# treangenlab/komb

Hardware: AMD Instinct MI355X
Metric: peeled edges/sec (k-truss) (higher is better)
Workload: dtype int32

## Files before the change

include/komb_accel.h:

```cpp
#ifndef KOMB_ACCEL_H
#define KOMB_ACCEL_H

#include <stdint.h>

#ifdef __cplusplus
extern "C" {
#endif

#define KOMB_ACCEL_ABI_VERSION 7

typedef enum komb_status {
    KOMB_OK          =  0,
    KOMB_ERR_ARG     = -1,
    KOMB_ERR_DEVICE  = -2,
    KOMB_ERR_NOMEM   = -3,
    KOMB_ERR_LIMIT   = -4,
    KOMB_ERR_STATE   = -5
} komb_status;

typedef struct komb_ctx komb_ctx;

typedef struct komb_opts {
    int32_t device;
    int32_t verbosity;
// ... 2 lines not shown
#define KOMB_CREATE_NULL_STREAM 1
#define KOMB_CREATE_NO_WARMUP   2
#define KOMB_CREATE_WARM_UPLOAD 4

typedef struct komb_stats {
    int64_t nv, ne;
    int64_t triangles;
    int64_t sum_deg_sq;
    int64_t wedge_items;
    int64_t oriented_items;
    int32_t max_degree, max_coreness, max_trussness;
    int32_t core_levels, core_subrounds;
    int32_t core_launches, truss_tail_runs;
    int32_t truss_levels, truss_subrounds;
    int32_t truss_scans, truss_launches;
    double  ms_build;
    double  ms_core;
    double  ms_orient;
    double  ms_tri_count;
    double  ms_tri_fill;
    double  ms_compact;
    double  ms_support;
    double  ms_allreduce;
    double  ms_peel;
    double  ms_gather;
    double  ms_corea;
    double  ms_tail;
    int64_t core_local_items, truss_local_items;
    int32_t core_local_units, core_local_sweeps;
    int32_t truss_local_units, truss_local_sweeps;
    double  ms_core_local;
    double  ms_truss_local;
    double  ms_sort;
    int64_t tri_records;
    int32_t index_layout;
    int32_t shard_exchanges;
    double  ms_exchange;
    int64_t exchange_words;
    double  ms_build_h2d;
    double  ms_build_relabel;
    double  ms_prepare;
    int32_t truss_prepared;
    int32_t engine_flags;
    double  ms_prep_vertex;
    double  ms_prep_edges;
    double  ms_prep_rows;
    int32_t stream_retries;
    int32_t reserved0;
} komb_stats;
#define KOMB_ENGINE_LOCAL_FINISH 1
#define KOMB_ENGINE_LDS_TAIL     2
#define KOMB_ENGINE_SHARD_PEEL   4
#define KOMB_ENGINE_TWO_PASS     8

komb_ctx   *komb_create(const komb_opts *opts);
void        komb_destroy(komb_ctx *ctx);
const char *komb_last_error(const komb_ctx *ctx);
int         komb_abi_version(void);
int         komb_set_option(komb_ctx *ctx, const char *name, const char *value);

int komb_graph_from_edges(komb_ctx *ctx, int64_t nv, int64_t n_raw,
                          const int64_t *uv_pairs);

int komb_graph_from_csr(komb_ctx *ctx, int64_t nv, const int64_t *rowptr,
                        const int32_t *col);

int komb_graph_info(komb_ctx *ctx, int64_t *nv, int64_t *ne);

int komb_graph_get_csr(komb_ctx *ctx, int64_t *rowptr, int32_t *col);

int komb_core_run(komb_ctx *ctx);
typedef int (*komb_allreduce_fn)(void *user, void *device_u32, int64_t count);
int komb_core_run_sharded(komb_ctx *ctx, int32_t rank, int32_t world, komb_allreduce_fn allreduce, void *user);
int komb_core_fetch(komb_ctx *ctx, int32_t *degree , int32_t *coreness );
int komb_degree_coreness(komb_ctx *ctx, int32_t *degree, int32_t *coreness);

int komb_onion_run(komb_ctx *ctx);
int komb_onion_fetch(komb_ctx *ctx, int32_t *layer , int32_t *coreness );
int komb_onion_info(komb_ctx *ctx, int64_t *n_layers, int32_t *max_coreness, double *ms);

#define KOMB_COMP_CORE   0
#define KOMB_COMP_TRUSS  1
#define KOMB_COMP_K_MAX (-1)
int komb_components_run(komb_ctx *ctx, int32_t kind, int32_t k);
int komb_components_fetch(komb_ctx *ctx, int32_t *label , int32_t *size );
int komb_components_info(komb_ctx *ctx, int32_t *kind, int32_t *k_used, int64_t *n_members,
                         int64_t *n_components, int64_t *largest, double *ms);

#define KOMB_COMM_K_MAX (-1)
int komb_truss_communities_run(komb_ctx *ctx, int32_t k);
int komb_truss_communities_fetch(komb_ctx *ctx, int32_t *label , int32_t *size );
int komb_truss_communities_fetch_vertices(komb_ctx *ctx, int32_t *n_comm );
int komb_truss_communities_info(komb_ctx *ctx, int32_t *k_used, int64_t *n_member_edges, int64_t *n_communities,
                                int64_t *largest, int64_t *n_multi_vertices, double *ms);

int komb_truss_run(komb_ctx *ctx, const uint8_t *vmask);
int komb_truss_prepare(komb_ctx *ctx);
int komb_truss_unprepare(komb_ctx *ctx);
int komb_truss_run_sharded(komb_ctx *ctx, const uint8_t *vmask, int32_t rank, int32_t world,
                           komb_allreduce_fn allreduce, void *user);
int komb_set_shard_peel(komb_ctx *ctx, int32_t on);
int komb_truss_run_slice(komb_ctx *ctx, const uint8_t *vmask, int32_t rank, int32_t world);
int komb_truss_count(komb_ctx *ctx, int64_t *ne_sub);
int komb_truss_fetch(komb_ctx *ctx, int32_t *eu, int32_t *ev, int32_t *truss);
int komb_truss_fetch_support(komb_ctx *ctx, int32_t *support);
int komb_trussness(komb_ctx *ctx, const uint8_t *vmask, int64_t *ne_out,
// ... 21 lines not shown
```

komb_amd/api.py:

```python
import ctypes
import os

import numpy as np

from . import _lib
from ._lib import KombOpts, KombStats, as_c, ptr


class KombError(RuntimeError):
    def __init__(self, code, msg):
        super().__init__(f"komb_accel error {code}: {msg}")
        self.code = code


def gen_hug_edges(nv, n_cliques, alpha=2.6, seed=42):
    lib = _lib.load()
    n_raw = lib.komb_gen_hug_edges(nv, n_cliques, alpha, seed, None)
    if n_raw < 0:
        raise ValueError("komb_gen_hug_edges: bad arguments")
    uv = np.empty((n_raw, 2), dtype=np.int64)
    got = lib.komb_gen_hug_edges(nv, n_cliques, alpha, seed, ptr(uv))
    assert got == n_raw
    return uv


FORWARD_ENV_OPTIONS = False
OPTION_NAMES = ("FINISH", "LOCAL_LIMIT", "LOCAL_ITEMS", "LOCAL_DENSITY", "LOCAL_DEFER_CHUNKS", "TAIL", "CORE_TAIL", "INDEX",
                "REC_CAP", "OWN_DENSE_CAP", "NO_OWN_DENSE", "NO_REC_SCRATCH", "NO_FIRST_QUEUE", "FULL_CAPS", "PREP_ROW_STAGE", "RETIRE_EVERY", "SHARD_ENGINE",
                "TRI_DEBUG", "POOL_DEBUG", "BUILD_DEBUG", "LOCAL_DEBUG", "TAIL_DEBUG", "COMP_SAMPLE", "COMM_SHORT", "COMM_HEAVY", "POISON")

SENTINEL_I32 = -0x5A5A5A5B


def _out_i32(n):
    return np.full(n, SENTINEL_I32, dtype=np.int32)


def _out_f64(n):
    return np.full(n, np.nan, dtype=np.float64)


class KombAccel:
    def __init__(self, device=0, verbosity=0, flags=0):
        self._lib = _lib.load()
        opts = KombOpts(device=device, verbosity=verbosity)
        opts.reserved[0] = flags
        self._ctx = self._lib.komb_create(ctypes.byref(opts))
        if not self._ctx:
            raise MemoryError("komb_create failed")
        self.device = device
        self.nv = -1
        self.ne = 0
        self._forwarded = {}

    def set_option(self, name, value):
        v = None if value is None else str(value).encode()
        self._check(self._lib.komb_set_option(self._ctx, name.encode(), v))

    def _sync_env_options(self):
        if not FORWARD_ENV_OPTIONS:
            return
        for name in OPTION_NAMES:
            v = os.environ.get("KOMB_" + name)
            if name == "INDEX" and os.environ.get("KOMB_TWO_PASS"):
                v = "two_pass"
            if name == "SHARD_ENGINE" and v is None:
                v = os.environ.get("KOMB_SHARD_PEEL")
            if self._forwarded.get(name) != v:
                self.set_option(name, v)
                self._forwarded[name] = v

    def close(self):
        if getattr(self, "_ctx", None):
            self._lib.komb_destroy(self._ctx)
            self._ctx = None

    def __del__(self):
        self.close()

    def __enter__(self):
# ... 203 lines not shown
```

komb_amd/csrc/api.cpp:

```cpp
#include "common.h"

#include <cerrno>
#include <cmath>
#include <cstdlib>
#include <cstring>
#include <memory>
#include <new>
#include <vector>

using namespace komb;

namespace {

int require_device(komb_ctx *ctx)
{
    if (!ctx) return KOMB_ERR_ARG;
    if (!ctx->device_ok) {
        if (ctx->err.empty()) ctx->err = "no usable HIP device";
        return KOMB_ERR_DEVICE;
    }
    KOMB_HIP(ctx, hipSetDevice(ctx->device));
    ctx->err.clear();
    return KOMB_OK;
}

}

extern "C" {

int komb_abi_version(void) { return KOMB_ACCEL_ABI_VERSION; }

komb_ctx *komb_create(const komb_opts *opts)
{
    komb_ctx *ctx = new (std::nothrow) komb_ctx();
    if (!ctx) return nullptr;
    if (opts) ctx->opts = *opts;
    ctx->device = ctx->opts.device;
    int ndev = 0;
    hipError_t e = hipGetDeviceCount(&ndev);
    if (e != hipSuccess || ndev <= 0) {
        ctx->err = std::string("no usable HIP device: ") + (e != hipSuccess ? hipGetErrorString(e) : "device count is 0");
        (void)hipGetLastError();
        return ctx;
    }
    if (ctx->device < 0 || ctx->device >= ndev) {
        ctx->err = "device ordinal out of range";
        return ctx;
    }
    e = hipSetDevice(ctx->device);
    if (e == hipSuccess) e = hipHostMalloc((void **)&ctx->h_ctrl, 2 * sizeof(PeelCtrl), hipHostMallocDefault);
    if (e == hipSuccess) e = hipHostMalloc((void **)&ctx->h_local, 2 * sizeof(LocalCtrl), hipHostMallocDefault);
    if (e == hipSuccess) e = hipHostMalloc(&ctx->h_stage, kStageBytes, hipHostMallocDefault);
    ctx->stream = nullptr;
    if (e == hipSuccess && !(ctx->opts.reserved[0] & KOMB_CREATE_NULL_STREAM)) { e = hipStreamCreate(&ctx->stream); ctx->own_stream = e == hipSuccess; }
    if (e == hipSuccess && !ctx->timer.init()) e = hipErrorUnknown;
    if (e != hipSuccess) {
        ctx->err = std::string("device initialisation failed: ") + hipGetErrorString(e);
        return ctx;
    }
    ctx->device_ok = true;
    if (!(ctx->opts.reserved[0] & KOMB_CREATE_NO_WARMUP)) warm_up(ctx);
    return ctx;
}

void komb_destroy(komb_ctx *ctx)
{
    if (!ctx) return;
    if (ctx->device_ok) {
        (void)hipSetDevice(ctx->device);
        graph_free(ctx);
        stager_free(ctx);
        ctx->pool.clear();
        ctx->timer.destroy();
        if (ctx->own_stream && ctx->stream) (void)hipStreamDestroy(ctx->stream);
        if (ctx->h_ctrl) (void)hipHostFree(ctx->h_ctrl);
        if (ctx->h_local) (void)hipHostFree(ctx->h_local);
        if (ctx->h_stage) (void)hipHostFree(ctx->h_stage);
    }
    delete ctx;
}

const char *komb_last_error(const komb_ctx *ctx) { return ctx ? ctx->err.c_str() : "null context"; }

int komb_graph_from_edges(komb_ctx *ctx, int64_t nv, int64_t n_raw, const int64_t *uv_pairs)
{
    KOMB_TRY(require_device(ctx));
    return graph_from_edges(ctx, nv, n_raw, uv_pairs);
}

int komb_graph_from_csr(komb_ctx *ctx, int64_t nv, const int64_t *rowptr, const int32_t *col)
{
    KOMB_TRY(require_device(ctx));
    return graph_from_csr(ctx, nv, rowptr, col);
}

int komb_graph_info(komb_ctx *ctx, int64_t *nv, int64_t *ne)
{
    if (!ctx) return KOMB_ERR_ARG;
    if (ctx->nv < 0) KOMB_FAIL(ctx, KOMB_ERR_STATE, "komb_graph_info: no graph loaded");
    if (nv) *nv = ctx->nv;
    if (ne) *ne = ctx->ne;
    return KOMB_OK;
}

int komb_graph_get_csr(komb_ctx *ctx, int64_t *rowptr, int32_t *col)
{
    KOMB_TRY(require_device(ctx));
    if (ctx->nv < 0) KOMB_FAIL(ctx, KOMB_ERR_STATE, "komb_graph_get_csr: no graph loaded");
    if (!rowptr || (ctx->ne > 0 && !col)) KOMB_FAIL(ctx, KOMB_ERR_ARG, "komb_graph_get_csr: null output");
    std::vector<uint32_t> rp((size_t)ctx->nv + 1);
    KOMB_HIP(ctx, hipMemcpy(rp.data(), ctx->d_o_rowptr, rp.size() * sizeof(uint32_t), hipMemcpyDeviceToHost));
    for (size_t i = 0; i < rp.size(); ++i) rowptr[i] = (int64_t)rp[i];
    if (ctx->ne > 0)
        KOMB_HIP(ctx, hipMemcpy(col, ctx->d_o_col, (size_t)(2 * ctx->ne) * sizeof(int32_t), hipMemcpyDeviceToHost));
    return KOMB_OK;
}

int komb_core_run(komb_ctx *ctx)
{
    KOMB_TRY(require_device(ctx));
    return core_run(ctx);
}

int komb_core_run_sharded(komb_ctx *ctx, int32_t rank, int32_t world, komb_allreduce_fn allreduce, void *user)
{
    KOMB_TRY(require_device(ctx));
// ... 298 lines not shown
```

komb_amd/csrc/common.h:

```cpp
#pragma once

#include <hip/hip_runtime.h>

#include <chrono>
#include <cstddef>
#include <cstdint>
#include <cstdio>
#include <cstdlib>
#include <cstring>
#include <map>
#include <string>
#include <vector>

#include "komb_accel.h"

#include <roctracer/roctx.h>

namespace komb {

struct Range {
    explicit Range(const char *name) { (void)roctxRangePushA(name); }
    ~Range() { (void)roctxRangePop(); }
    void next(const char *name) { (void)roctxRangePop(); (void)roctxRangePushA(name); }
    Range(const Range &) = delete;
// ... 139 lines not shown
        }
        blocks.push_back({q, bytes, true});
        if (poison.on) { e = poison.fill(q, bytes); if (e != hipSuccess) { put(q); return e; } }
        *out = q;
        return hipSuccess;
    }
    void put(void *p)
    {
        if (!p) return;
        for (auto &b : blocks) if (b.p == p) { b.used = false; return; }
    }
    size_t unused_bytes() const
    {
        size_t t = 0;
        for (const auto &b : blocks) if (!b.used) t += b.bytes;
        return t;
    }
    void trim()
    {
        std::vector<Block> keep;
        for (auto &b : blocks) { if (b.used) keep.push_back(b); else (void)hipFree(b.p); }
        blocks.swap(keep);
    }
    void clear()
    {
        for (auto &b : blocks) (void)hipFree(b.p);
        blocks.clear();
    }
};

struct TrussPrep {
    bool valid = false;
    int64_t nv = 0, ne = 0;
    int32_t  *o2i = nullptr, *i2o = nullptr;
    uint32_t *orow = nullptr;
    int32_t  *ocol = nullptr, *osrc = nullptr;
    uint32_t *e2k = nullptr;
    uint4    *vline = nullptr;
    void     *wtasks = nullptr;
    int64_t   n_wtasks = 0;
    int64_t   own_bound = 0;
    double    ms = 0.0;
    double    ms_part[4] = {0, 0, 0, 0};
};

struct komb_ctx {
    komb_opts opts{};
    DevPool pool;
    std::string err;
    bool device_ok = false;
    int device = 0;
    hipStream_t stream = nullptr;
    bool own_stream = false;
    komb::Timer timer;
    std::map<std::string, std::string> options;

    int64_t nv = -1, ne = 0;
    uint32_t *d_o_rowptr = nullptr;
    int32_t  *d_o_col = nullptr;
    TrussPrep prep;

    int32_t *d_deg = nullptr;
    int32_t *d_core = nullptr;
    bool core_done = false;

    int32_t *d_onion_layer = nullptr;
    int32_t *d_onion_core = nullptr;
    int64_t onion_layers = 0;
    int32_t onion_max_core = 0;
    double onion_ms = 0.0;
    bool onion_done = false;

    int32_t *d_comp_label = nullptr;
    int32_t *d_comp_size = nullptr;
    int32_t comp_kind = 0, comp_k = 0;
    int64_t comp_members = 0, comp_count = 0, comp_largest = 0;
    double comp_ms = 0.0;
    bool comp_done = false;

    int32_t *d_comm_label = nullptr;
    int32_t *d_comm_size = nullptr;
    int32_t *d_comm_ncomm = nullptr;
    int32_t comm_k = 0;
    int64_t comm_members = 0, comm_count = 0, comm_largest = 0, comm_multi = 0;
    double comm_ms = 0.0, comm_ms_vertices = 0.0;
    bool comm_done = false, comm_v_ready = false;

    int64_t t_ne = -1;
    int32_t *d_t_eu = nullptr, *d_t_ev = nullptr, *d_t_truss = nullptr, *d_t_sup = nullptr;
    uint2 *d_t_slice = nullptr;
    uint32_t t_k_lo = 0, t_k_hi = 0;
    bool t_sup_ready = false;
    bool t_own_edges = false;
    int32_t *d_ceu = nullptr, *d_cev = nullptr;
    bool truss_done = false;
    int slice_rank = 0, slice_world = 1;
    bool shard_peel = false;
    struct { int64_t nv = -1, m = -1; unsigned long long own_cap = 0, rec_cap = 0; } cap_hint;

    komb::PeelCtrl *h_ctrl = nullptr;
    komb::LocalCtrl *h_local = nullptr;
    void *h_stage = nullptr;
    struct H2DStager *stager = nullptr;

    komb_stats stats{};
};
// ... 232 lines not shown
```

komb_amd/csrc/ktruss.hip:

```cpp
#include "peel_dev.h"
#include "truss_tail.h"
#include "local_dev.h"
#include "shard_dev.h"

#include <algorithm>
#include <cstdlib>
#include <cstring>

#include "truss_line.h"
#include "truss_tri.h"
#include "truss_wedge.h"
#include "truss_index.h"
#include "truss_gather.h"

namespace komb {

namespace {

struct TrussProblem {
    static constexpr bool kChain = false;
    static constexpr bool kSingleStep = false;
    uint32_t units;
    const uint2 *off2;
    const int2 *inc;
// ... 542 lines not shown
#else
    TrussProblem P{(uint32_t)m, d_off2, d_inc, d_sup, d_stamp, d_st8, retire_every};
#endif
    TailBufs T{};
    if (fin == FIN_LDS && tail_limit) {
        KOMB_HIP(ctx, bufs.alloc(&T.vmap, (size_t)nv));
        KOMB_HIP(ctx, bufs.alloc(&T.cnt, 64));
        KOMB_HIP(ctx, bufs.alloc(&T.vlist, (size_t)kTailMaxV));
        KOMB_HIP(ctx, bufs.alloc(&T.rows, (size_t)kTailMaxV * kTailRowWords));
        KOMB_HIP(ctx, bufs.alloc(&T.pair, (size_t)tail_limit));
        KOMB_HIP(ctx, bufs.alloc(&T.sup, (size_t)tail_limit));
        KOMB_HIP(ctx, bufs.alloc(&T.gid, (size_t)tail_limit));
        KOMB_HIP(ctx, bufs.alloc(&T.gid_by_rank, (size_t)tail_limit));
        KOMB_HIP(ctx, bufs.alloc(&T.pair_by_rank, (size_t)tail_limit));
        KOMB_HIP(ctx, bufs.alloc(&T.truss_by_rank, (size_t)tail_limit));
        KOMB_HIP(ctx, bufs.alloc(&T.spill[0], (size_t)tail_limit));
        KOMB_HIP(ctx, bufs.alloc(&T.spill[1], (size_t)tail_limit));
        T.max_edges = tail_limit;
    }
    auto run_tail = [&](const int32_t *list, uint32_t n_in) -> int {
        KOMB_HIP(ctx, hipMemsetAsync(T.vmap, 0, (size_t)nv * sizeof(int32_t), s));
        KOMB_HIP(ctx, hipMemsetAsync(T.cnt, 0, 64 * sizeof(uint32_t), s));
        KOMB_HIP(ctx, hipMemsetAsync(T.rows, 0, (size_t)kTailMaxV * kTailRowWords * sizeof(unsigned long long), s));
        const int g = grid_for(n_in, kBlock, 256);
        const bool dbg = ctx_flag(ctx, "TAIL_DEBUG");
        hipEvent_t ev[3] = {nullptr, nullptr, nullptr};
        for (auto &e : ev) (void)hipEventCreate(&e);
        (void)hipEventRecord(ev[0], s);
        k_tail_mark<<<g, kBlock, 0, s>>>(list, n_in, d_sup, d_stamp, d_osrc, d_ocol, T);
        k_tail_number<<<1, kTailMaxV, 0, s>>>(T);
        k_tail_rows<<<g, kBlock, 0, s>>>(list, n_in, d_sup, d_stamp, d_osrc, d_ocol, T);
        (void)hipEventRecord(ev[1], s);
        k_truss_tail<<<1, 1024, 0, s>>>(d_ctrl, T, d_truss);
        (void)hipEventRecord(ev[2], s);
        KOMB_HIP(ctx, d2h(ctx, &ctx->h_ctrl[0], d_ctrl, sizeof(PeelCtrl)));
        ++st.truss_tail_runs;
        float m0 = 0, m1 = 0, m2 = 0;
        (void)hipEventElapsedTime(&m0, ctx->timer.a, ev[0]); (void)hipEventElapsedTime(&m1, ev[0], ev[1]); (void)hipEventElapsedTime(&m2, ev[1], ev[2]);
        for (auto &e : ev) (void)hipEventDestroy(e);
        st.ms_tail += (double)m1 + (double)m2;
        if (dbg) {
            uint32_t h[16];
            KOMB_HIP(ctx, d2h(ctx, h, T.cnt, sizeof(h)));
            fprintf(stderr, "komb tail: %u vertices, %u edges, %s; general engine before it %.1f us, setup %.1f us, tail kernel %.1f us\n",
                    h[0], h[1], ctx->h_ctrl[0].done == 1 ? "done" : "refused", m0 * 1000.f, m1 * 1000.f, m2 * 1000.f);
#ifdef KOMB_TAIL_TIMERS
            fprintf(stderr, "komb tail: us in kernel: load %.1f ranks %.1f supports %.1f scan %.1f mark %.1f triangles %.1f retire %.1f results %.1f\n",
                    h[14] / 100.0, h[15] / 100.0, h[8] / 100.0, h[9] / 100.0, h[10] / 100.0, h[11] / 100.0, h[12] / 100.0, h[13] / 100.0);
#endif
        }
        return KOMB_OK;
    };
    const int gp = peel_grid(m);
    auto run_local = [&]() -> int {
        const PeelCtrl hc = ctx->h_ctrl[0];
        EventSet evs;
        hipEvent_t ev[2] = {nullptr, nullptr};
        for (auto &e : ev) KOMB_HIP(ctx, evs.make(&e));
        (void)hipEventRecord(ev[0], s);
        LocalStats ls;
        const int lrc = local_finish(ctx, bufs, hc, d_ctrl, (uint32_t)m, d_stamp, d_sup, Q.live[hc.live_sel],
            (uint32_t)kWave * TrussLocal::kU, sizeof(uint2), local_item_limit(ctx, kTrussLocalItems), local_density_limit(ctx, kTrussLocalDensity), true, 2, d_truss,
            [&](const LocalGraph &lg, const int32_t *num, void *items, PeelCtrl *d_cctrl, int32_t launch) {
                TrussCollect C{(uint32_t)m, d_off2, d_inc, d_stamp, num, lg.off, lg.cur, (uint2 *)items};
                PeelQueues Qc = Q;
                Qc.rlevel = nullptr;
                k_peel_step<TrussCollect><<<gp, kPeelBlock, 0, s>>>(d_cctrl, d_grp, Qc, C, launch);
            },
            [&](const LocalGraph &lg, void *items, uint64_t total_items, LocalCtrl *d_lctrl, uint32_t *d_cnt, int *nl) -> int {
                return local_fixpoint(ctx, d_lctrl, d_cnt, lg, TrussLocal{(const uint2 *)items}, total_items, nl);
            },
            &ls, [](const LocalGraph &) {});
        (void)hipEventRecord(ev[1], s);
        (void)hipEventSynchronize(ev[1]);
        float ms = 0.f;
        (void)hipEventElapsedTime(&ms, ev[0], ev[1]);
        KOMB_TRY(lrc);
        if (ls.refused) { ctx->h_ctrl[0].done = 0; ctx->h_ctrl[0].tail_limit = ls.new_limit; return KOMB_OK; }
        st.truss_local_units = (int32_t)ls.units; st.truss_local_sweeps = ls.sweeps; st.truss_local_items = (int64_t)ls.items;
        st.ms_truss_local = (double)ms;
        PeelCtrl fin_c = hc;
        fin_c.done = 1; fin_c.remaining = 0;
        fin_c.n_levels += (int32_t)ls.levels;
        fin_c.max_level = ls.max_val > fin_c.max_level ? ls.max_val : fin_c.max_level;
        ctx->h_ctrl[0] = fin_c;
        return KOMB_OK;
    };
    ctx->timer.start(s);
    if (!peel_inited) {
        peel_ctrl_pre(s, d_grp);
        k_peel_init<<<grid_for(m, kBlock, 1024), kBlock, 0, s>>>(m, d_off, d_off2, d_sup, d_stamp, d_st8, d_grp + kInitOff);
    }
    peel_ctrl_init(s, d_ctrl, d_grp, (uint32_t)m, tail_limit);
    int launches = 0, rc = KOMB_OK;
    st.truss_tail_runs = 0; st.ms_tail = 0.0;
    st.truss_local_units = 0; st.truss_local_sweeps = 0; st.truss_local_items = 0; st.ms_truss_local = 0.0;
    st.shard_exchanges = 0; st.ms_exchange = 0.0; st.exchange_words = 0;
    if (shard_peel_on) {
        uint32_t iw[2] = {0u, 0u};
        KOMB_HIP(ctx, d2h(ctx, iw, d_grp + kInitOff, sizeof(iw)));
        ShardTruss SP{(uint32_t)m, d_off2, d_inc, d_sup, d_stamp, 0u, 0u};
        shard_bounds((uint64_t)m, rank, world, &SP.lo, &SP.hi);
        ShardStats ss;
        rc = shard_peel(ctx, bufs, SP, d_sup, (uint32_t)m, iw[0], (int32_t)iw[1], rank, world, fn, user, Q, d_ctrl,
                        [&](int32_t launch) { k_peel_step<ShardTruss><<<gp, kPeelBlock, 0, s>>>(d_ctrl, d_grp, Q, SP, launch); },
                        fin == FIN_LOCAL ? tail_limit : 0u, [&]() -> int { return run_local(); }, &ss);
        st.shard_exchanges = (int32_t)ss.exchanges; st.ms_exchange = ss.ms_exchange; st.exchange_words = ss.words;
        launches = ss.launches;
        PeelCtrl fc{};
        fc.done = rc == KOMB_OK ? 1 : 2; fc.n_levels = ss.levels; fc.n_rounds = ss.rounds; fc.n_scans = ss.scans; fc.max_level = ss.max_level;
        ctx->h_ctrl[0] = fc;
    } else if (whole_peel_finish) {
        rc = d2h(ctx, &ctx->h_ctrl[0], d_ctrl, sizeof(PeelCtrl)) == hipSuccess ? KOMB_OK : KOMB_ERR_DEVICE;
        if (rc == KOMB_OK && !ctx->h_ctrl[0].done) rc = (fin == FIN_LOCAL) ? run_local() : run_tail(nullptr, (uint32_t)m);
    } else {
        ctx->h_ctrl[0].done = 0;
    }
    for (int guard = 0; rc == KOMB_OK && ctx->h_ctrl[0].done != 1 && ctx->h_ctrl[0].done != 2 && guard < 64; ++guard) {
        if (ctx->h_ctrl[0].done == 3) {
            const PeelCtrl &c = ctx->h_ctrl[0];
            if (fin == FIN_LOCAL) rc = run_local();
            else rc = c.live_mode ? run_tail(Q.live[c.live_sel], c.live_count) : run_tail(nullptr, (uint32_t)m);
            continue;
        }
        int batch = 0;
        rc = drive_peel(ctx, d_ctrl, m, [&](int32_t launch) {
            k_peel_step<TrussProblem><<<gp, kPeelBlock, 0, s>>>(d_ctrl, d_grp, Q, P, launch);
        }, &batch);
        launches += batch;
    }
    st.ms_peel = ctx->timer.stop(s);
    KOMB_TRY(rc);
#ifdef KOMB_STEP_TIMERS
    {
        const PeelCtrl &c = ctx->h_ctrl[0];
        const double n = c.pad1[6] ? (double)c.pad1[6] : 1.0;
        fprintf(stderr, "komb step timers (block 0, %u small multi-workgroup PROCESS steps), us per step: ctrl %.2f queue+slice %.2f items %.2f flush %.2f barrier %.2f ticket %.2f\n",
                c.pad1[6], c.pad1[0] / n / 100.0, c.pad1[1] / n / 100.0, c.pad1[2] / n / 100.0, c.pad1[3] / n / 100.0, c.pad1[4] / n / 100.0, c.pad1[5] / n / 100.0);
    }
#endif
    if (ctx->h_ctrl[0].done != 1) KOMB_FAIL(ctx, KOMB_ERR_DEVICE, "k-truss peel ended in an inconsistent state");
    if (ctx->h_ctrl[0].max_retire_gap > retire_every)
        KOMB_FAIL(ctx, KOMB_ERR_DEVICE, "k-truss peel: %d sub-rounds passed without a RETIRE step (period %d): edge state codes may have wrapped",
                  ctx->h_ctrl[0].max_retire_gap, retire_every);
    st.engine_flags = (layout == IDX_TWO_PASS ? KOMB_ENGINE_TWO_PASS : 0) | (shard_peel_on ? KOMB_ENGINE_SHARD_PEEL : 0) |
                      (st.truss_local_units ? KOMB_ENGINE_LOCAL_FINISH : 0) | (st.truss_tail_runs ? KOMB_ENGINE_LDS_TAIL : 0);
    st.truss_levels = ctx->h_ctrl[0].n_levels;
    st.truss_subrounds = ctx->h_ctrl[0].n_rounds;
    st.truss_launches = launches;
    st.truss_scans = ctx->h_ctrl[0].n_scans;
    st.max_trussness = ctx->h_ctrl[0].max_level + 2;
    for (int i = 0; i < 2; ++i) { bufs.release(Q.light[i]); bufs.release(Q.heavy[i]); bufs.release(Q.live[i]); }
    bufs.release(Q.code);
    bufs.release(d_sup); bufs.release(d_inc);

    phase.next("truss: canonical gather");
    ctx->timer.start(s);
    KOMB_HIP(ctx, ctx->pool.get((void **)&ctx->d_t_truss, (size_t)m * sizeof(int32_t)));
    uint32_t k_lo = 0, k_hi = (uint32_t)m;
    if (!vmask_host) {
        ctx->d_t_eu = ctx->d_ceu; ctx->d_t_ev = ctx->d_cev;
        ctx->t_own_edges = false;
        if (ctx->slice_world > 1) {
            shard_bounds((uint64_t)m, ctx->slice_rank, ctx->slice_world, &k_lo, &k_hi);
#ifndef KOMB_TEST_SKIP_SLICE_ZERO
            if (k_lo) KOMB_HIP(ctx, hipMemsetAsync(ctx->d_t_truss, 0, (size_t)k_lo * sizeof(int32_t), s));
            if (k_hi < (uint32_t)m) KOMB_HIP(ctx, hipMemsetAsync(ctx->d_t_truss + k_hi, 0, ((size_t)m - k_hi) * sizeof(int32_t), s));
#endif
        }
    } else {
        ctx->t_own_edges = true;
        KOMB_HIP(ctx, ctx->pool.get((void **)&ctx->d_t_eu, (size_t)m * sizeof(int32_t)));
        KOMB_HIP(ctx, ctx->pool.get((void **)&ctx->d_t_ev, (size_t)m * sizeof(int32_t)));
        KOMB_TRY(edge_list(ctx, sub.rowptr, sub.col, sub.nv, sub.vold, ctx->d_t_eu, ctx->d_t_ev));
    }
    ctx->t_k_lo = k_lo; ctx->t_k_hi = k_hi;
    k_truss_results<<<grid_for(m), kBlock, 0, s>>>(d_stamp, Q.rlevel, d_truss, tp->e2k, m, k_lo, k_hi, ctx->d_t_truss);
    ctx->d_t_slice = d_off2;
    bufs.detach(d_off2);
    ctx->t_sup_ready = false;
    if (vmask_host) {
        ctx->t_ne = m;
        KOMB_HIP(ctx, ctx->pool.get((void **)&ctx->d_t_sup, (size_t)m * sizeof(int32_t)));
        k_scatter_len<<<grid_for(m), kBlock, 0, s>>>(ctx->d_t_slice, tp->e2k, m, 0u, (uint32_t)m, ctx->d_t_sup);
        ctx->t_sup_ready = true;
    }
    st.ms_gather = ctx->timer.stop(s);
    if (ctx_flag(ctx, "POOL_DEBUG")) {
        size_t held = 0;
        for (const auto &b : ctx->pool.blocks) held += b.bytes;
        fprintf(stderr, "komb pool: %zu blocks, %.2f GB held, %zu hipMalloc calls so far (%.1f ms inside them), %zu trims\n", ctx->pool.blocks.size(), held / 1e9, ctx->pool.n_malloc, ctx->pool.ms_malloc, ctx->pool.n_trim);
    }
    if (vmask_host) KOMB_HIP(ctx, hipStreamSynchronize(s));
    ctx->t_ne = m;
    ctx->truss_done = true;
    return KOMB_OK;
}

}
```

komb_amd/csrc/local_dev.h:

```cpp
#pragma once

#include "peel_dev.h"

namespace komb {

constexpr int kLocBlock = 512;
constexpr int kLocWaves = kLocBlock / kWave;
constexpr int kLocHB = 4096;
constexpr int kLocBins = kLocHB / kLocBlock;
constexpr int kCntWays = 8;
constexpr int kCntWords = (5 * kCntWays + 5) * 32;
constexpr int kCntTimerWords = 6 * 12 * 2;
constexpr int kHvU = 8;
constexpr uint32_t kKeyBins = 4096;
constexpr uint32_t kMedMax = 2048;
constexpr int kGiantWin = 8;
constexpr uint32_t kGiantChunk = 8192;
constexpr int kLocBatch = 6;


struct LocalGraph {
    uint32_t n, nh;
    uint32_t *off;
    int32_t *val;
// ... 679 lines not shown
    if (per_sweep) { sw.resize(1); if (evs.make(&sw[0]) == hipSuccess) (void)hipEventRecord(sw[0], s); }
    while (!finished && (uint64_t)launches < max_launches && k < 0x3FFFFFF0) {
        for (int i = 0; i < kLocBatch; ++i) {
            ++k;
            if (g.flags & kLocUseList) k_local_list<<<list_grid, kListBlock, 0, s>>>(d_ctrl, d_cnt, g, k);
            k_local_step<P><<<grid, kLocBlock, 0, s>>>(d_ctrl, d_cnt, g, p, k, full_thr); ++launches;
            if (g.nchunk && (g.flags & kLocDeferNotify)) k_local_giant_notify<P><<<(int)std::min<uint32_t>(g.nchunk, 1024u), kLocBlock, 0, s>>>(d_ctrl, g, p, k);
            if (per_sweep && sw.size() < 600) { hipEvent_t e2 = nullptr; if (evs.make(&e2) == hipSuccess) { (void)hipEventRecord(e2, s); sw.push_back(e2); } }
        }
        if (hipMemcpyAsync(&h[slot], d_ctrl, sizeof(LocalCtrl), hipMemcpyDeviceToHost, s) != hipSuccess ||
            hipEventRecord(ev[slot], s) != hipSuccess) { status = KOMB_ERR_DEVICE; break; }
        if (have_prev) {
            if (hipEventSynchronize(ev[slot ^ 1]) != hipSuccess) { status = KOMB_ERR_DEVICE; break; }
            if (h[slot ^ 1].done) finished = true;
            else if ((int32_t)h[slot ^ 1].spare[0] == seen_iters) { stuck = true; finished = true; }
            seen_iters = (int32_t)h[slot ^ 1].spare[0];
        }
        have_prev = true;
        slot ^= 1;
    }
    hipError_t e = hipStreamSynchronize(s);
    if (per_sweep) {
        fprintf(stderr, "komb local sweeps (us):");
        for (size_t i = 1; i < sw.size(); ++i) { float ms = 0.f; (void)hipEventElapsedTime(&ms, sw[i - 1], sw[i]); fprintf(stderr, " %.0f", ms * 1e3f); }
        fprintf(stderr, "\n");
    }
    if (launches_out) *launches_out = launches;
    if (status != KOMB_OK || e != hipSuccess)
        KOMB_FAIL(ctx, KOMB_ERR_DEVICE, "local fixed point: HIP failure (%s)", hipGetErrorString(e));
    if (stuck) KOMB_FAIL(ctx, KOMB_ERR_DEVICE, "local fixed point: the sweeps make no progress (sweep %d)", (int)seen_iters);
    return KOMB_OK;
}

static __global__ __launch_bounds__(kBlock) void k_local_zero(uint32_t *a, uint32_t na, uint32_t *b, uint32_t nb, uint32_t *c, uint32_t nc,
                                                       uint32_t *d, uint32_t nd, uint32_t *e, uint32_t ne)
{
    const uint32_t t = blockIdx.x * kBlock + threadIdx.x, step = gridDim.x * kBlock;
    for (uint32_t i = t; i < na; i += step) a[i] = 0u;
    for (uint32_t i = t; i < nb; i += step) b[i] = 0u;
    for (uint32_t i = t; i < nc; i += step) c[i] = 0u;
    for (uint32_t i = t; i < nd; i += step) d[i] = 0u;
    for (uint32_t i = t; i < ne; i += step) e[i] = 0u;
}

struct LocalStats {
    uint32_t units = 0, heavy = 0, levels = 0;
    int32_t max_val = 0;
    int sweeps = 0, launches = 0;
    uint64_t items = 0, evals = 0;
    bool refused = false;
    uint32_t new_limit = 0;
};

template <class LaunchCollect, class RunFix, class AfterNumber>
int local_finish(komb_ctx *ctx, DevBufs &bufs, const PeelCtrl &hc, PeelCtrl *d_ctrl, uint32_t units, const int32_t *marker,
                 const int32_t *key, const int32_t *live_list, uint32_t light_max, size_t item_bytes, uint64_t item_limit, uint32_t max_density, bool use_list, int32_t add, int32_t *out,
                 LaunchCollect &&launch_collect, RunFix &&run_fix, LocalStats *ls, AfterNumber &&after_number)
{
    hipStream_t s = ctx->stream;
    const uint32_t n = hc.remaining;
    if (n == 0) KOMB_FAIL(ctx, KOMB_ERR_STATE, "local finish: nothing left to hand over");
    const bool dbg = ctx_opt(ctx, "LOCAL_DEBUG") != nullptr;
    EventSet evs;
    hipEvent_t ev[5] = {nullptr, nullptr, nullptr, nullptr, nullptr};
    if (dbg) for (auto &e : ev) (void)evs.make(&e);
    auto stamp = [&](int i) { if (dbg) (void)hipEventRecord(ev[i], s); };
    stamp(0);
    const int32_t *list = hc.live_mode ? live_list : nullptr;
    const uint32_t n_in = hc.live_mode ? hc.live_count : units;
    LocalGraph g{};
    int32_t *d_num = nullptr;
    LocalCtrl *d_lctrl = nullptr;
    PeelCtrl *d_cctrl = nullptr;
    uint32_t *d_present = nullptr;
    const size_t present_words = ((size_t)units >> 5) + 2 > kFinWords ? ((size_t)units >> 5) + 2 : (size_t)kFinWords;
    KOMB_HIP(ctx, bufs.alloc(&d_num, (size_t)units));
    KOMB_HIP(ctx, bufs.alloc(&g.off, (size_t)n + 1));
    KOMB_HIP(ctx, bufs.alloc(&g.len, (size_t)n + 1));
    KOMB_HIP(ctx, bufs.alloc(&g.val, (size_t)n));
    KOMB_HIP(ctx, bufs.alloc(&g.mark[0], (size_t)n));
    KOMB_HIP(ctx, bufs.alloc(&g.mark[1], (size_t)n));
    KOMB_HIP(ctx, bufs.alloc(&g.gid, (size_t)n));
    KOMB_HIP(ctx, bufs.alloc(&g.cur, (size_t)n));
    KOMB_HIP(ctx, bufs.alloc(&g.list, (size_t)n));
    KOMB_HIP(ctx, bufs.alloc(&g.giant, (size_t)n));
    KOMB_HIP(ctx, bufs.alloc(&g.khist, (size_t)kKeyBins));
    KOMB_HIP(ctx, bufs.alloc(&d_lctrl, 1));
    uint32_t *d_cnt = nullptr;
    KOMB_HIP(ctx, bufs.alloc(&d_cnt, (size_t)kCntWords + kCntTimerWords));
    KOMB_HIP(ctx, bufs.alloc(&d_cctrl, 1));
    KOMB_HIP(ctx, bufs.alloc(&d_present, present_words));
    static_assert(sizeof(LocalCtrl) % sizeof(uint32_t) == 0, "LocalCtrl is zeroed word by word");
    if (present_words > 0xFFFFFFFFull) KOMB_FAIL(ctx, KOMB_ERR_LIMIT, "local finish: %zu presence words", present_words);
    k_local_zero<<<64, kBlock, 0, s>>>(g.khist, kKeyBins, d_cnt, (uint32_t)(kCntWords + kCntTimerWords), (uint32_t *)d_lctrl, (uint32_t)(sizeof(LocalCtrl) / sizeof(uint32_t)),
                                       g.len + n, 1u, d_present, (uint32_t)present_words);
    void *d_items = nullptr;
    auto release_all = [&]() {
        bufs.release(d_items); bufs.release(d_num); bufs.release(g.off); bufs.release(g.len); bufs.release(g.val);
        bufs.release(g.mark[0]); bufs.release(g.mark[1]); bufs.release(g.gid); bufs.release(g.list); bufs.release(g.giant); bufs.release(g.gchunk); bufs.release(g.gacc); bufs.release(g.gwin); bufs.release(g.gnote);
        bufs.release(g.khist); bufs.release(g.cur); bufs.release(d_lctrl); bufs.release(d_cnt); bufs.release(d_cctrl); bufs.release(d_present);
    };
    g.n = n; g.nh = 0; g.ng = 0; g.nchunk = 0;
    int64_t gb = ((int64_t)n_in + kNumBlock - 1) / kNumBlock;
    k_local_number<<<(int)(gb < 1 ? 1 : (gb > 1024 ? 1024 : gb)), kNumBlock, 0, s>>>(list, n_in, n, marker, key, light_max, d_num, g, d_lctrl);
    LocalCtrl hl{};
    std::vector<uint32_t> kh(kKeyBins);
    if (ctx->h_stage && sizeof(LocalCtrl) + kKeyBins * sizeof(uint32_t) <= kStageBytes) {
        char *st8 = (char *)ctx->h_stage;
        KOMB_HIP(ctx, hipMemcpyAsync(st8, d_lctrl, sizeof(LocalCtrl), hipMemcpyDeviceToHost, s));
        KOMB_HIP(ctx, hipMemcpyAsync(st8 + sizeof(LocalCtrl), g.khist, kKeyBins * sizeof(uint32_t), hipMemcpyDeviceToHost, s));
// ... 19 lines not shown
        if (ls) { ls->refused = true; ls->new_limit = (uint32_t)nl; }
        release_all();
        return KOMB_OK;
    }
    KOMB_TRY(prim_exclusive_sum_u32(ctx, g.len, g.off, (int64_t)n + 1));
    const uint32_t total = (uint32_t)hl.key_sum;
    g.nh = hl.n_heavy;
    g.ng = hl.n_giant;
    g.nchunk = hl.n_chunk;
    uint32_t defer_chunks = kLocDeferChunks;
    if (const char *e = ctx_opt(ctx, "LOCAL_DEFER_CHUNKS")) defer_chunks = (uint32_t)strtoul(e, nullptr, 10);
    g.flags = (use_list ? kLocUseList : 0u) | (g.nchunk >= defer_chunks && g.nchunk > 0 ? kLocDeferNotify : 0u);
#ifdef KOMB_DEBUG_SWITCHES
    if (const char *e = getenv("KOMB_LOCAL_MODE")) g.flags = (uint32_t)atoi(e);
#endif
    if (g.ng) {
        KOMB_HIP(ctx, bufs.alloc(&g.gchunk, (size_t)g.nchunk));
        KOMB_HIP(ctx, bufs.alloc(&g.gacc, (size_t)g.ng));
        KOMB_HIP(ctx, bufs.alloc(&g.gwin, (size_t)g.ng * kGiantWin));
        KOMB_HIP(ctx, bufs.alloc(&g.gnote, (size_t)g.ng));
        k_local_chunks<<<(int)(g.ng > 1024u ? 1024u : g.ng), kBlock, 0, s>>>(g);
    }
    int32_t K = 0x7FFFFFFF;
    {
        uint64_t ge = 0;
        for (int32_t k = (int32_t)kKeyBins - 1; k >= 0; --k) {
            ge += kh[(size_t)k];
            if (ge >= (uint64_t)k) { if (k < (int32_t)kKeyBins - 1) K = k; break; }
        }
    }
    stamp(1);
    after_number(g);
    KOMB_HIP(ctx, bufs.alloc((unsigned char **)&d_items, (size_t)total * item_bytes));

    peel_collect_ctrl(s, d_cctrl, d_ctrl);
    PeelCtrl hcc{};
    int32_t cl = 1;
    for (int guard = 0; guard < 16 && hcc.done == 0; ++guard) {
        for (int i = 0; i < 3; ++i) launch_collect(g, d_num, d_items, d_cctrl, cl++);
        KOMB_HIP(ctx, d2h(ctx, &hcc, d_cctrl, sizeof(PeelCtrl)));
        cl = hcc.seq;
    }
    if (hcc.done != 1) KOMB_FAIL(ctx, KOMB_ERR_DEVICE, "local finish: collect pass did not complete (state %d)", hcc.done);
    int64_t gn = ((int64_t)n + kBlock - 1) / kBlock;
    const int grid_n = (int)(gn > 1024 ? 1024 : gn);
    k_local_check<<<grid_n, kBlock, 0, s>>>(g, d_lctrl);
    if (K != 0x7FFFFFFF) k_local_clamp<<<grid_n, kBlock, 0, s>>>(g, K);
    stamp(2);

    int launches = 0;
    KOMB_TRY(run_fix(g, d_items, (uint64_t)total, d_lctrl, d_cnt, &launches));
    stamp(3);
    k_local_finish<<<grid_n, kBlock, 0, s>>>(g, add, out, d_present, d_lctrl);
    k_local_levels<<<(int)(present_words / kBlock + 1 > 256 ? 256 : present_words / kBlock + 1), kBlock, 0, s>>>(d_present, (uint32_t)present_words, d_cnt, d_lctrl);
    stamp(4);
    KOMB_HIP(ctx, d2h(ctx, &hl, d_lctrl, sizeof(LocalCtrl)));
    if (dbg) {
        float t[4] = {0, 0, 0, 0};
        for (int i = 0; i < 4; ++i) (void)hipEventElapsedTime(&t[i], ev[i], ev[i + 1]);
        fprintf(stderr, "komb local finish: %u units (%u heavy, %u of them long; bound %d), %u items; number+scan %.1f us, collect %.1f us, %d sweeps (%d launches, %u evaluations) %.1f us, scatter %.1f us\n",
                n, g.nh, g.ng, K == 0x7FFFFFFF ? -1 : K, total, t[0] * 1e3f, t[1] * 1e3f, hl.iters, launches, hl.evals, t[2] * 1e3f, t[3] * 1e3f);
    }
#ifdef KOMB_LOCAL_TIMERS
    {
        unsigned long long tm[72];
        KOMB_HIP(ctx, d2h(ctx, tm, d_cnt + kCntWords, sizeof(tm)));
        for (int sw = 0; sw < 6; ++sw) {
            const unsigned long long *t = tm + sw * 12;
            const double nwv = t[10] ? (double)t[10] : 1.0;
            fprintf(stderr, "komb local timers, sweep %d (%llu waves), us per wave: hscan %.1f medium %.1f workgroup %.1f setup %.1f load+count %.1f search %.1f notify %.1f; "
                            "batches/wave %.2f groups/wave %.2f; slowest wave %.1f us\n",
                    sw == 0 ? 1 : sw * 4, t[10], t[0] / nwv / 100.0, t[1] / nwv / 100.0, t[2] / nwv / 100.0, t[3] / nwv / 100.0, t[4] / nwv / 100.0, t[5] / nwv / 100.0,
                    t[6] / nwv / 100.0, t[7] / nwv, t[8] / nwv, t[9] / 100.0);
        }
    }
#endif
    if (hl.bad) KOMB_FAIL(ctx, KOMB_ERR_DEVICE, "local finish: %u consistency failures in the compact index", hl.bad);
    if (!hl.done) KOMB_FAIL(ctx, KOMB_ERR_DEVICE, "local finish: launch budget exhausted before the fixed point");
    if (ls) {
        ls->units = n; ls->heavy = g.nh; ls->levels = hl.levels; ls->max_val = hl.max_val;
        ls->sweeps = hl.iters; ls->launches = launches; ls->items = total; ls->evals = hl.evals;
    }
    release_all();
    return KOMB_OK;
}

}
```

komb_amd/csrc/truss_gather.h:

```cpp
#pragma once

#include "peel_dev.h"

namespace komb {

namespace {

__global__ __launch_bounds__(kBlock) void k_truss_results(const int32_t *__restrict__ stamp, const int32_t *__restrict__ rlevel,
                                                         const int32_t *__restrict__ truss,
                                                         const uint32_t *__restrict__ e2k, int64_t m, uint32_t k_lo, uint32_t k_hi,
                                                         int32_t *__restrict__ tr_out)
{
    for (int64_t e = (int64_t)blockIdx.x * kBlock + threadIdx.x; e < m; e += (int64_t)gridDim.x * kBlock) {
        const int32_t s = stamp[e];
        const int32_t t = marker_alive(s) ? truss[e] : rlevel[s] + 2;
        const uint32_t k = e2k[e];
        if (k - k_lo < k_hi - k_lo) tr_out[k] = t;
    }
}

__global__ __launch_bounds__(kBlock) void k_scatter_len(const uint2 *__restrict__ off2, const uint32_t *__restrict__ e2k, int64_t m,
                                                       uint32_t k_lo, uint32_t k_hi, int32_t *__restrict__ out)
{
    for (int64_t e = (int64_t)blockIdx.x * kBlock + threadIdx.x; e < m; e += (int64_t)gridDim.x * kBlock) {
        const uint32_t k = e2k[e];
        if (k - k_lo < k_hi - k_lo) out[k] = (int32_t)off2[e].y;
    }
}

}

}
```

Before: 4.115 billion.

## Overlap peeled-edge results gather with local finish on a side stream

```diff
diff --git a/include/komb_accel.h b/include/komb_accel.h
--- a/include/komb_accel.h
+++ b/include/komb_accel.h
@@ -78,6 +78,7 @@
 #define KOMB_ENGINE_LDS_TAIL     2
 #define KOMB_ENGINE_SHARD_PEEL   4
 #define KOMB_ENGINE_TWO_PASS     8
+#define KOMB_ENGINE_RESULTS_OVERLAP 16
 
 komb_ctx   *komb_create(const komb_opts *opts);
 void        komb_destroy(komb_ctx *ctx);
diff --git a/komb_amd/api.py b/komb_amd/api.py
--- a/komb_amd/api.py
+++ b/komb_amd/api.py
@@ -25,7 +25,7 @@
 
 
 FORWARD_ENV_OPTIONS = False
-OPTION_NAMES = ("FINISH", "LOCAL_LIMIT", "LOCAL_ITEMS", "LOCAL_DENSITY", "LOCAL_DEFER_CHUNKS", "TAIL", "CORE_TAIL", "INDEX",
+OPTION_NAMES = ("FINISH", "LOCAL_LIMIT", "LOCAL_ITEMS", "LOCAL_DENSITY", "LOCAL_DEFER_CHUNKS", "TAIL", "CORE_TAIL", "INDEX", "RESULTS",
                 "REC_CAP", "OWN_DENSE_CAP", "NO_OWN_DENSE", "NO_REC_SCRATCH", "NO_FIRST_QUEUE", "FULL_CAPS", "PREP_ROW_STAGE", "RETIRE_EVERY", "SHARD_ENGINE",
                 "TRI_DEBUG", "POOL_DEBUG", "BUILD_DEBUG", "LOCAL_DEBUG", "TAIL_DEBUG", "COMP_SAMPLE", "COMM_SHORT", "COMM_HEAVY", "POISON")
 
diff --git a/komb_amd/csrc/api.cpp b/komb_amd/csrc/api.cpp
--- a/komb_amd/csrc/api.cpp
+++ b/komb_amd/csrc/api.cpp
@@ -54,6 +54,11 @@
     ctx->stream = nullptr;
     if (e == hipSuccess && !(ctx->opts.reserved[0] & KOMB_CREATE_NULL_STREAM)) { e = hipStreamCreate(&ctx->stream); ctx->own_stream = e == hipSuccess; }
     if (e == hipSuccess && !ctx->timer.init()) e = hipErrorUnknown;
+    if (e == hipSuccess && ctx->own_stream) {
+        e = hipStreamCreateWithFlags(&ctx->side, hipStreamNonBlocking);
+        if (e == hipSuccess) e = hipEventCreateWithFlags(&ctx->side_ev[0], hipEventDisableTiming);
+        for (int i = 1; i < 5 && e == hipSuccess; ++i) e = hipEventCreate(&ctx->side_ev[i]);
+    }
     if (e != hipSuccess) {
         ctx->err = std::string("device initialisation failed: ") + hipGetErrorString(e);
         return ctx;
@@ -72,6 +77,8 @@
         stager_free(ctx);
         ctx->pool.clear();
         ctx->timer.destroy();
+        for (auto &ev : ctx->side_ev) if (ev) (void)hipEventDestroy(ev);
+        if (ctx->side) (void)hipStreamDestroy(ctx->side);
         if (ctx->own_stream && ctx->stream) (void)hipStreamDestroy(ctx->stream);
         if (ctx->h_ctrl) (void)hipHostFree(ctx->h_ctrl);
         if (ctx->h_local) (void)hipHostFree(ctx->h_local);
diff --git a/komb_amd/csrc/common.h b/komb_amd/csrc/common.h
--- a/komb_amd/csrc/common.h
+++ b/komb_amd/csrc/common.h
@@ -215,6 +215,8 @@
     int device = 0;
     hipStream_t stream = nullptr;
     bool own_stream = false;
+    hipStream_t side = nullptr;
+    hipEvent_t side_ev[5] = {nullptr, nullptr, nullptr, nullptr, nullptr};
     komb::Timer timer;
     std::map<std::string, std::string> options;
 
diff --git a/komb_amd/csrc/ktruss.hip b/komb_amd/csrc/ktruss.hip
--- a/komb_amd/csrc/ktruss.hip
+++ b/komb_amd/csrc/ktruss.hip
@@ -618,6 +618,56 @@
         return KOMB_OK;
     };
     const int gp = peel_grid(m);
+    bool overlap_ok = ctx->side != nullptr && fin == FIN_LOCAL && !shard_peel_on;
+    if (const char *rs = ctx_opt(ctx, "RESULTS")) {
+        if (!strcmp(rs, "serial")) overlap_ok = false;
+        else if (strcmp(rs, "overlap")) KOMB_FAIL(ctx, KOMB_ERR_ARG, "option RESULTS=%s: expected overlap or serial", rs);
+    }
+    uint32_t k_lo = 0, k_hi = (uint32_t)m;
+    bool out_ready = false;
+    auto result_array = [&]() -> int {
+        if (out_ready) return KOMB_OK;
+        KOMB_HIP(ctx, ctx->pool.get((void **)&ctx->d_t_truss, (size_t)m * sizeof(int32_t)));
+        out_ready = true;
+        if (!vmask_host && ctx->slice_world > 1) {
+            shard_bounds((uint64_t)m, ctx->slice_rank, ctx->slice_world, &k_lo, &k_hi);
+#ifndef KOMB_TEST_SKIP_SLICE_ZERO
+            if (k_lo) KOMB_HIP(ctx, hipMemsetAsync(ctx->d_t_truss, 0, (size_t)k_lo * sizeof(int32_t), s));
+            if (k_hi < (uint32_t)m) KOMB_HIP(ctx, hipMemsetAsync(ctx->d_t_truss + k_hi, 0, ((size_t)m - k_hi) * sizeof(int32_t), s));
+#endif
+        }
+        return KOMB_OK;
+    };
+    struct SideJoin {
+        komb_ctx *c;
+        bool started = false, joined = false;
+        hipError_t join()
+        {
+            if (!started || joined) return hipSuccess;
+            joined = true;
+            return hipStreamWaitEvent(c->stream, c->side_ev[2], 0);
+        }
+        ~SideJoin() { if (started) { (void)join(); (void)hipStreamSynchronize(c->side); } }
+    } side{ctx};
+    int side_rc = KOMB_OK;
+    auto start_bulk = [&]() -> int {
+        KOMB_TRY(result_array());
+        KOMB_HIP(ctx, hipEventRecord(ctx->side_ev[0], s));
+        KOMB_HIP(ctx, hipStreamWaitEvent(ctx->side, ctx->side_ev[0], 0));
+        KOMB_HIP(ctx, hipEventRecord(ctx->side_ev[1], ctx->side));
+        k_truss_results_peeled<<<(int)std::min<int64_t>(kPeeledGrid, grid_for(m)), kBlock, 0, ctx->side>>>(d_stamp, Q.rlevel, tp->e2k, m, k_lo, k_hi, ctx->d_t_truss);
+        const hipError_t e = hipEventRecord(ctx->side_ev[2], ctx->side);
+        side.started = true;
+        KOMB_HIP(ctx, e);
+        KOMB_HIP(ctx, hipGetLastError());
+        return KOMB_OK;
+    };
+    auto remainder_results = [&](const LocalGraph &lg) -> int {
+        KOMB_HIP(ctx, hipEventRecord(ctx->side_ev[3], s));
+        k_truss_results_units<<<grid_for(lg.n), kBlock, 0, s>>>(lg.gid, lg.n, d_truss, tp->e2k, k_lo, k_hi, ctx->d_t_truss);
+        KOMB_HIP(ctx, hipEventRecord(ctx->side_ev[4], s));
+        return KOMB_OK;
+    };
     auto run_local = [&]() -> int {
         const PeelCtrl hc = ctx->h_ctrl[0];
         EventSet evs;
@@ -636,12 +686,14 @@
             [&](const LocalGraph &lg, void *items, uint64_t total_items, LocalCtrl *d_lctrl, uint32_t *d_cnt, int *nl) -> int {
                 return local_fixpoint(ctx, d_lctrl, d_cnt, lg, TrussLocal{(const uint2 *)items}, total_items, nl);
             },
-            &ls, [](const LocalGraph &) {});
+            &ls, [&](const LocalGraph &) { if (overlap_ok && !side.started) side_rc = start_bulk(); },
+            [&](const LocalGraph &lg) { if (side.started && side_rc == KOMB_OK) side_rc = remainder_results(lg); });
         (void)hipEventRecord(ev[1], s);
         (void)hipEventSynchronize(ev[1]);
         float ms = 0.f;
         (void)hipEventElapsedTime(&ms, ev[0], ev[1]);
         KOMB_TRY(lrc);
+        KOMB_TRY(side_rc);
         if (ls.refused) { ctx->h_ctrl[0].done = 0; ctx->h_ctrl[0].tail_limit = ls.new_limit; return KOMB_OK; }
         st.truss_local_units = (int32_t)ls.units; st.truss_local_sweeps = ls.sweeps; st.truss_local_items = (int64_t)ls.items;
         st.ms_truss_local = (double)ms;
@@ -695,6 +747,7 @@
         }, &batch);
         launches += batch;
     }
+    if (side.join() != hipSuccess && rc == KOMB_OK) { ctx->err = "k-truss: joining the side stream's results pass failed"; rc = KOMB_ERR_DEVICE; }
     st.ms_peel = ctx->timer.stop(s);
     KOMB_TRY(rc);
 #ifdef KOMB_STEP_TIMERS
@@ -710,7 +763,8 @@
         KOMB_FAIL(ctx, KOMB_ERR_DEVICE, "k-truss peel: %d sub-rounds passed without a RETIRE step (period %d): edge state codes may have wrapped",
                   ctx->h_ctrl[0].max_retire_gap, retire_every);
     st.engine_flags = (layout == IDX_TWO_PASS ? KOMB_ENGINE_TWO_PASS : 0) | (shard_peel_on ? KOMB_ENGINE_SHARD_PEEL : 0) |
-                      (st.truss_local_units ? KOMB_ENGINE_LOCAL_FINISH : 0) | (st.truss_tail_runs ? KOMB_ENGINE_LDS_TAIL : 0);
+                      (st.truss_local_units ? KOMB_ENGINE_LOCAL_FINISH : 0) | (st.truss_tail_runs ? KOMB_ENGINE_LDS_TAIL : 0) |
+                      (side.started ? KOMB_ENGINE_RESULTS_OVERLAP : 0);
     st.truss_levels = ctx->h_ctrl[0].n_levels;
     st.truss_subrounds = ctx->h_ctrl[0].n_rounds;
     st.truss_launches = launches;
@@ -722,18 +776,10 @@
 
     phase.next("truss: canonical gather");
     ctx->timer.start(s);
-    KOMB_HIP(ctx, ctx->pool.get((void **)&ctx->d_t_truss, (size_t)m * sizeof(int32_t)));
-    uint32_t k_lo = 0, k_hi = (uint32_t)m;
+    KOMB_TRY(result_array());
     if (!vmask_host) {
         ctx->d_t_eu = ctx->d_ceu; ctx->d_t_ev = ctx->d_cev;
         ctx->t_own_edges = false;
-        if (ctx->slice_world > 1) {
-            shard_bounds((uint64_t)m, ctx->slice_rank, ctx->slice_world, &k_lo, &k_hi);
-#ifndef KOMB_TEST_SKIP_SLICE_ZERO
-            if (k_lo) KOMB_HIP(ctx, hipMemsetAsync(ctx->d_t_truss, 0, (size_t)k_lo * sizeof(int32_t), s));
-            if (k_hi < (uint32_t)m) KOMB_HIP(ctx, hipMemsetAsync(ctx->d_t_truss + k_hi, 0, ((size_t)m - k_hi) * sizeof(int32_t), s));
-#endif
-        }
     } else {
         ctx->t_own_edges = true;
         KOMB_HIP(ctx, ctx->pool.get((void **)&ctx->d_t_eu, (size_t)m * sizeof(int32_t)));
@@ -741,7 +787,7 @@
         KOMB_TRY(edge_list(ctx, sub.rowptr, sub.col, sub.nv, sub.vold, ctx->d_t_eu, ctx->d_t_ev));
     }
     ctx->t_k_lo = k_lo; ctx->t_k_hi = k_hi;
-    k_truss_results<<<grid_for(m), kBlock, 0, s>>>(d_stamp, Q.rlevel, d_truss, tp->e2k, m, k_lo, k_hi, ctx->d_t_truss);
+    if (!side.started) k_truss_results<<<grid_for(m), kBlock, 0, s>>>(d_stamp, Q.rlevel, d_truss, tp->e2k, m, k_lo, k_hi, ctx->d_t_truss);
     ctx->d_t_slice = d_off2;
     bufs.detach(d_off2);
     ctx->t_sup_ready = false;
@@ -752,6 +798,12 @@
         ctx->t_sup_ready = true;
     }
     st.ms_gather = ctx->timer.stop(s);
+    if (side.started) {
+        float mb = 0.f, mr = 0.f;
+        (void)hipEventElapsedTime(&mb, ctx->side_ev[1], ctx->side_ev[2]);
+        (void)hipEventElapsedTime(&mr, ctx->side_ev[3], ctx->side_ev[4]);
+        st.ms_gather += (double)mb + (double)mr;
+    }
     if (ctx_flag(ctx, "POOL_DEBUG")) {
         size_t held = 0;
         for (const auto &b : ctx->pool.blocks) held += b.bytes;
diff --git a/komb_amd/csrc/local_dev.h b/komb_amd/csrc/local_dev.h
--- a/komb_amd/csrc/local_dev.h
+++ b/komb_amd/csrc/local_dev.h
@@ -755,10 +755,12 @@
     uint32_t new_limit = 0;
 };
 
-template <class LaunchCollect, class RunFix, class AfterNumber>
+inline void local_no_hook(const LocalGraph &) {}
+template <class LaunchCollect, class RunFix, class AfterNumber, class AfterScatter = void (*)(const LocalGraph &)>
 int local_finish(komb_ctx *ctx, DevBufs &bufs, const PeelCtrl &hc, PeelCtrl *d_ctrl, uint32_t units, const int32_t *marker,
                  const int32_t *key, const int32_t *live_list, uint32_t light_max, size_t item_bytes, uint64_t item_limit, uint32_t max_density, bool use_list, int32_t add, int32_t *out,
-                 LaunchCollect &&launch_collect, RunFix &&run_fix, LocalStats *ls, AfterNumber &&after_number)
+                 LaunchCollect &&launch_collect, RunFix &&run_fix, LocalStats *ls, AfterNumber &&after_number,
+                 AfterScatter &&after_scatter = &local_no_hook)
 {
     hipStream_t s = ctx->stream;
     const uint32_t n = hc.remaining;
@@ -884,6 +886,7 @@
     KOMB_TRY(run_fix(g, d_items, (uint64_t)total, d_lctrl, d_cnt, &launches));
     stamp(3);
     k_local_finish<<<grid_n, kBlock, 0, s>>>(g, add, out, d_present, d_lctrl);
+    after_scatter(g);
     k_local_levels<<<(int)(present_words / kBlock + 1 > 256 ? 256 : present_words / kBlock + 1), kBlock, 0, s>>>(d_present, (uint32_t)present_words, d_cnt, d_lctrl);
     stamp(4);
     KOMB_HIP(ctx, d2h(ctx, &hl, d_lctrl, sizeof(LocalCtrl)));
diff --git a/komb_amd/csrc/truss_gather.h b/komb_amd/csrc/truss_gather.h
--- a/komb_amd/csrc/truss_gather.h
+++ b/komb_amd/csrc/truss_gather.h
@@ -19,6 +19,41 @@
     }
 }
 
+constexpr int kPeeledGrid = 1024;
+constexpr int kPeeledU = 4;
+__global__ __launch_bounds__(kBlock) void k_truss_results_peeled(const int32_t *__restrict__ stamp, const int32_t *__restrict__ rlevel,
+                                                                const uint32_t *__restrict__ e2k, int64_t m, uint32_t k_lo, uint32_t k_hi,
+                                                                int32_t *__restrict__ tr_out)
+{
+    const int64_t step = (int64_t)gridDim.x * kBlock;
+    for (int64_t e0 = (int64_t)blockIdx.x * kBlock + threadIdx.x; e0 < m; e0 += step * kPeeledU) {
+        int32_t s[kPeeledU];
+        uint32_t k[kPeeledU];
+#pragma unroll
+        for (int x = 0; x < kPeeledU; ++x) {
+            const int64_t e = e0 + (int64_t)x * step;
+            s[x] = e < m ? stamp[e] : kAlive;
+            k[x] = e < m ? e2k[e] : 0u;
+        }
+        int32_t t[kPeeledU];
+#pragma unroll
+        for (int x = 0; x < kPeeledU; ++x) t[x] = marker_alive(s[x]) ? 0 : rlevel[s[x]] + 2;
+#pragma unroll
+        for (int x = 0; x < kPeeledU; ++x)
+            if (!marker_alive(s[x]) && k[x] - k_lo < k_hi - k_lo) tr_out[k[x]] = t[x];
+    }
+}
+__global__ __launch_bounds__(kBlock) void k_truss_results_units(const int32_t *__restrict__ gid, uint32_t n, const int32_t *__restrict__ truss,
+                                                               const uint32_t *__restrict__ e2k, uint32_t k_lo, uint32_t k_hi,
+                                                               int32_t *__restrict__ tr_out)
+{
+    for (uint32_t i = blockIdx.x * kBlock + threadIdx.x; i < n; i += gridDim.x * kBlock) {
+        const int32_t e = gid[i];
+        const uint32_t k = e2k[e];
+        if (k - k_lo < k_hi - k_lo) tr_out[k] = truss[e];
+    }
+}
+
 __global__ __launch_bounds__(kBlock) void k_scatter_len(const uint2 *__restrict__ off2, const uint32_t *__restrict__ e2k, int64_t m,
                                                        uint32_t k_lo, uint32_t k_hi, int32_t *__restrict__ out)
 {
```

Result: no change. 4.101 billion (-0.4%).
